# aff3ct/dvbs2

Measured on AMD Instinct MI355X. Metric: info_bits_per_s (N=64800 LDPC NMS 10-ite), higher is better.
Workload: dtype f32

## Files before the change

dvbs2_amd/csrc/dvbs2hip_api.hip:

```cpp
#include "dvbs2hip_handle.h"
#include "ldpc_dispatch.h"
#include "dvbs2_tables_gen.h"
#include <climits>
#include <new>

using namespace dvbs2;

namespace dvbs2 {
thread_local std::string g_create_error;

const char *modcod_name_by_pls(int b0_b6)
{
    for (int i = 0; i < DVBS2_N_MODCODS; i++) {
        int v = 0;
        for (int k = 0; k < 7; k++) v = v << 1 | (dvbs2_modcod_rows[i].pls[k] & 1);
        if (v == b0_b6) return dvbs2_modcod_rows[i].name;
    }
    return nullptr;
}

int pl_frame_by_pls(int b0_b6)
{
    for (int i = 0; i < DVBS2_N_MODCODS; i++) {
        const dvbs2_modcod_row &r = dvbs2_modcod_rows[i];
// ... 217 lines not shown
    const_cast<dvbs2hip_t *>(h)->ldpc_name = ldpc_choice_name(ldpc_choice(h, h->max_frames));
    return h->ldpc_name.c_str();
}

int dvbs2hip_reset(dvbs2hip_t *h)
{
    if (!h) return DVBS2HIP_EINVAL;
    int r = dvbs2hip_filter_reset(h);
    if (r) return r;
    if ((r = dvbs2hip_estimate_pilots_reset(h))) return r;
    if ((r = dvbs2hip_bbframe_reset(h))) return r;
    return dvbs2hip_monitor_reset(h);
}

int dvbs2hip_set_ldpc_params(dvbs2hip_t *h, int32_t n_ite, float alpha, int32_t early_stop)
{
    if (!h) return DVBS2HIP_EINVAL;
    if (n_ite < 1) return fail(h, DVBS2HIP_EINVAL, "'n_ite' has to be greater than 0");
    if (!(alpha > 0.f)) return fail(h, DVBS2HIP_EINVAL, "'alpha' has to be greater than 0");
    h->n_ite = n_ite; h->alpha = alpha; h->early_stop = early_stop ? 1 : 0;
    return 0;
}

void *dvbs2hip_get_stream(dvbs2hip_t *h) { return h ? (void *)h->stream : nullptr; }

int dvbs2hip_synchronize(dvbs2hip_t *h)
{
    int r0 = enter(h); if (r0) return r0;
    HIPCHK(h, hipStreamSynchronize(h->stream));
    return lr_check_all(h);
}

int dvbs2hip_graph_begin(dvbs2hip_t *h)
{
    int r0 = enter(h); if (r0) return r0;
    if (h->capturing) return fail(h, DVBS2HIP_EINVAL, "a capture is already open on this handle");
    if (h->timing) return fail(h, DVBS2HIP_EINVAL, "the per-kernel timers are on: their events cannot be recorded into a graph (dvbs2hip_timing_enable(h, 0) first)");
    HIPCHK(h, hipStreamBeginCapture(h->stream, hipStreamCaptureModeThreadLocal));
    h->capturing = true;
    return 0;
}

int dvbs2hip_graph_end(dvbs2hip_t *h, int32_t *graph)
{
    if (!h || !graph) return DVBS2HIP_EINVAL;
    if (!h->capturing) return fail(h, DVBS2HIP_EINVAL, "no capture is open on this handle");
// ... 25 lines not shown
    if (graph < 0 || (size_t)graph >= h->graphs.size() || !h->graphs[(size_t)graph]) return fail(h, DVBS2HIP_EINVAL, "unknown graph");
    (void)hipGraphExecDestroy(h->graphs[(size_t)graph]);
    h->graphs[(size_t)graph] = nullptr;
    return 0;
}

int dvbs2hip_get_sizes(const dvbs2hip_t *h, dvbs2hip_sizes *o)
{
    if (!h || !o) return DVBS2HIP_EINVAL;
    o->N_ldpc = h->N_ldpc; o->K_ldpc = h->K_ldpc; o->K_bch = h->K_bch; o->bps = h->bps;
    o->N_xfec_sym = h->n_sym; o->pl_frame_sym = h->pl_frame; o->ldpc_edges = h->ldpc.E; o->ldpc_q = h->ldpc.q;
    return 0;
}

static int ldpc_dev(dvbs2hip_t *h, const LdpcChoice &ch, const float *Y, int8_t *CWD, int32_t *V, uint32_t *packed, float *post, int32_t *ites, int F, int32_t *info_out = nullptr,
                    uint8_t *bch_flag = nullptr, int8_t *cwd_bch = nullptr)
{
    if (!ch.error.empty()) return fail(h, DVBS2HIP_EUNSUPPORTED, ch.error);
    LdpcKParams p;
    memset(&p, 0, sizeof p);
    p.llr = Y; p.bits = V; p.packed = packed; p.cwd = CWD; p.post = post; p.ites = ites; p.gwork = h->d_gwork;
    p.info_out = info_out; p.info_prbs = h->bch.d_prbs_rw; p.K_info = h->K_bch;
    if (info_out && bch_flag) { p.syn_tab = h->d_syn_pos; p.info_prbs_s = h->d_prbs_s; p.syn_words = h->syn_words; p.syn_rows = h->syn_rows; p.bch_flag = bch_flag; p.cwd_bch = cwd_bch; }
    p.n_frames = F; p.n_ite = h->n_ite; p.early_stop = h->early_stop; p.alpha = h->alpha;
    if (h->ldpc_sched == DVBS2HIP_SCHED_NATURAL) {
        LdpcPlan &pl = h->ldpc;
        if (!h->d_nat_work || !pl.d_nat_tab || !pl.d_nat_haz) {
            const size_t bytes = ((size_t)h->max_frames + 63) / 64 * ldpc_nat_group_words(pl) * sizeof(float);
            if (!h->d_nat_work && dev_alloc(h, &h->d_nat_work, bytes, "natural-order LDPC: workspace of " + std::to_string(bytes) + " bytes does not fit")) return DVBS2HIP_ENOMEM;
            if (!pl.d_nat_tab && upload(h, &pl.d_nat_tab, pl.nat_tab)) { (void)dev_free(h, &pl.d_nat_tab); return DVBS2HIP_EHIP; }
            if (!pl.d_nat_haz && upload(h, &pl.d_nat_haz, pl.nat_haz)) { (void)dev_free(h, &pl.d_nat_haz); return DVBS2HIP_EHIP; }
        }
    }
    Timer tm(h, DVBS2HIP_K_LDPC);
    if (ch.takes_order) {
        void *dord;
        int r = ensure(h, B_ORDER, (size_t)F * 8, &dord);
        if (r) return r;
        HIPCHK(h, frame_order_launch(Y, (float *)dord + F, (uint32_t *)dord, F, h->N_ldpc, h->stream));
        p.order = (const uint32_t *)dord;
    }
    HIPCHK(h, ldpc_launch(h->ldpc, ch, p, h->d_nat_work, h->stream));
    return 0;
}

int dvbs2hip_ldpc_decode_siho_dev(dvbs2hip_t *h, const float *Y_N, int8_t *CWD, int32_t *V_K, int32_t F)
{
// ... 356 lines not shown
```

dvbs2_amd/csrc/dvbs2hip_handle.h:

```cpp
#pragma once
#include "dvbs2hip_internal.h"
#include <cmath>
#include <cstdio>
#include <cstdlib>
#include <cstring>
#include <algorithm>
#include <map>
#include <utility>

namespace dvbs2 {

extern thread_local std::string g_create_error;

struct DevBuf {
    void *p = nullptr;
    size_t bytes = 0;
};

template <typename T>
struct PingPong {
    T *p[2] = {nullptr, nullptr};
    int cur = 0;
    T *in() const { return p[cur]; }
    T *out() const { return p[cur ^ 1]; }
    void flip() { cur ^= 1; }
};

}

struct dvbs2hip_handle {
    int N_ldpc = 0, K_ldpc = 0, K_bch = 0, bps = 0, itl_cols = 1, itl_order = 0;
    int n_sym = 0, pl_frame = 0, max_frames = 1, device = 0;
    int n_ite = 50, early_stop = 1, implem = 0;
    float alpha = 1.f, code_rate = 0.f;
    int fir_T = 0, fir_osf = 1;
    bool fir_sym = false;
    hipStream_t stream = nullptr;
    bool own_stream = false;
    bool capturing = false;
    bool lat_lds_ok = false;
    bool comm_dead = false;
    int red_timeout_ms = 0;
    std::vector<hipGraphExec_t> graphs;
    int n_cus = 256;
    dvbs2::LdpcPlan ldpc;
    dvbs2::BchPlan bch;
    float *d_cstl = nullptr;
    uint8_t *d_pl_seq = nullptr;
    float *d_taps_rev = nullptr;
    uint16_t *d_fir_afrag = nullptr, *d_upfir_afrag = nullptr;
    dvbs2::PingPong<float> d_hist;
    void *d_hist_all = nullptr;
    size_t hist_stride = 0;
    float *d_taps = nullptr;
    dvbs2::PingPong<float> d_uphist;
    unsigned long long *d_ctr = nullptr;
// ... 341 lines not shown
```

dvbs2_amd/csrc/dvbs2hip_internal.h:

```cpp
#pragma once
#include <hip/hip_runtime.h>
#include <stdint.h>
#include <string>
#include <vector>
#include "../../include/dvbs2hip.h"
#include "ldpc_layer_table.h"

namespace dvbs2 {

#if defined(__HIPCC__)
__device__ __forceinline__ float hw_exp(float x) { return __builtin_amdgcn_exp2f(x * 1.44269504088896341f); }
__device__ __forceinline__ float hw_log(float x) { return __builtin_amdgcn_logf(x) * 0.693147180559945309f; }
#endif

typedef uint32_t LdpcEntry;
enum { LE_T0_MASK = 0x1FF, LE_SLOT_SHIFT = 9, LE_SLOT_MASK = 0xFF, LE_LDS = 1u << 17, LE_MASK0 = 1u << 18,
       LE_LVL_SHIFT = 19, LE_LVL_MASK = 3, LE_NULL = 1u << 21 };

struct LdpcGroup {
    uint32_t base;
    uint32_t lds;
};

constexpr int LDPC_Z = 360;
// ... 8 lines not shown
    int8_t *cwd;
    float *post;
    int32_t *ites;
    int32_t *info_out;
    const uint32_t *info_prbs;
    int32_t K_info;
    const uint32_t *syn_tab;
    const uint32_t *info_prbs_s;
    int32_t syn_words;
    int32_t syn_rows;
    uint8_t *bch_flag;
    int8_t *cwd_bch;
    float *gwork;
    const LdpcEntry *entries;
    const int32_t *layer_deg;
    const int32_t *layer_lvl;
    const LdpcGroup *groups;
    int32_t N, K, M, q, n_info, n_groups;
    int32_t ent_stride;
    int32_t lds_post_words;
    int32_t glb_post_words;
    int32_t gwork_words;
    int32_t n_frames, n_ite, early_stop;
    float alpha;
    const uint32_t *order;
    float spa_cap;
    int32_t inf_row;
    uint32_t *cu_ctr;
    struct {
        const uint32_t *tab;
        const uint32_t *atab;
        const uint32_t *rows;
        uint32_t st_base;
        uint32_t lds_junk;
        int32_t lds_bytes, pad;
        int32_t nl_info, nl, ng_info, ng;
    } w8;
};

struct LdpcPlan {
    int N = 0, K = 0, M = 0, q = 0, n_info = 0, n_groups = 0, E = 0;
    int deg_max = 0, ent_stride = 0;
    int lds_groups = 0;
    bool c2v_lds = false, hybrid = false;
    int lds_post_words = 0, glb_post_words = 0, gwork_words = 0;
    size_t lds_bytes = 0;
// ... 10 lines not shown
    int spa_rule = 0;
    int fast_deg = 0;
    bool fast_pad = false;
    int fast_inf_row = -1;
    int fast_mode = 0;
    std::vector<uint32_t> nat_tab, nat_haz;
    uint32_t *d_nat_tab = nullptr, *d_nat_haz = nullptr;
    bool fast_cu1 = false;
    int cu1_pairs = 0;
    bool fast_wg8 = false;
    bool w8_dups_in_lds = false;
    std::vector<uint32_t> w8_tab, w8_rows;
    uint32_t *d_w8_tab = nullptr, *d_w8_rows = nullptr;
    std::vector<uint32_t> w8_atab;
    uint32_t *d_w8_atab = nullptr;
    uint32_t w8_st_base = 0, w8_lds_junk = 0;
    int w8_lds_bytes = 0, w8_gwork_words = 0, w8_nl_info = 0, w8_nl = 0, w8_ng_info = 0, w8_ng = 0;
    int w8_park_moves = 0;
    uint32_t *d_cu_ctr = nullptr;
};
constexpr int LDPC_PROF_WORDS = 1024 * 64;
constexpr int LDPC_CU_CTR_WORDS = 4096 + 64;
constexpr int LDPC_FRAME_CTR = 4096;
#ifndef LDPC_SPA_AT16_MAXDEG
#define LDPC_SPA_AT16_MAXDEG 13
#endif
constexpr int LDPC_AT_LANES = 384;
constexpr float LDPC_SPA_CAP = 16.6355324f;
constexpr int LDPC_FAST_MAXC = 16;
__host__ __device__ __forceinline__ constexpr int ldpc_park_nr(int mode) { return mode == 5 ? 39 : 32; }
__host__ __device__ __forceinline__ constexpr int ldpc_park_nl(int mode) { return mode == 5 ? 15 : 14; }
__host__ __device__ __forceinline__ constexpr int ldpc_w8_kd(int deg) { return deg == 27 ? 6 : deg == 11 ? 3 : deg == 13 ? 6 : deg; }
#ifndef LDPC_CU1_HA_V
#define LDPC_CU1_HA_V 14
#endif
constexpr int LDPC_CU1_HA = LDPC_CU1_HA_V;
constexpr int LDPC_CU1_XCHG_BYTES = 2 * LDPC_Z * 8;
__host__ __device__ __forceinline__ constexpr int ldpc_cu1_nrg() { return 36; }
#ifndef LDPC_CU1_DEFAULT
#define LDPC_CU1_DEFAULT 0
#endif
#ifndef LDPC_CU1_SPA_DEFAULT
#define LDPC_CU1_SPA_DEFAULT 1
#endif
constexpr int LDPC_W8_MISC_BYTES = 96;
constexpr int LDPC_SYN_RED = 640;
constexpr int LDPC_SPA_MAXC = 6;
constexpr int NAT_AHEAD = 24;
constexpr int NAT_HAZ_WINDOW = NAT_AHEAD + 1;
size_t ldpc_nat_group_words(const LdpcPlan &pl);
hipError_t ldpc_wg8_launch(const LdpcPlan &pl, LdpcKParams p, hipStream_t s);
int ldpc_wg8_blocks_per_cu(const LdpcPlan &pl);

std::string ldpc_build_plan(LdpcPlan &pl, int N, int K, int n_rows, const int32_t *row_ptr,
                            const int32_t *addr, int lds_groups_req, size_t lds_limit_bytes, int spa_rule = 0, bool small_batch = false);

struct BchPlan {
    int m = 0, n = 0, t = 0, N = 0, K = 0;
    std::vector<uint16_t> exp_, log_;
    uint16_t *d_exp = nullptr, *d_log = nullptr;
    uint32_t *d_prbs = nullptr;
    uint32_t *d_prbs_rw = nullptr;
    std::vector<uint16_t> syn_tab;
    uint16_t *d_syn_tab = nullptr;
};
struct BchKParams {
    const int32_t *in_bits;
    const uint32_t *in_packed;
// ... 156 lines not shown
```

dvbs2_amd/csrc/k_ldpc_wg8.hip:

```cpp
#include "dvbs2hip_internal.h"
#include "ldpc_layer_table.h"
#include "ldpc_device.h"
#include <cstdio>
#include <cstdlib>
#include <vector>
#include <algorithm>
#include <type_traits>

#include "ldpc_det.h"
namespace dvbs2 {

constexpr int W8_NL = 9;
constexpr int W8_IO = 16;
constexpr uint32_t W8_OOB = ATAB_DROPPED;
__host__ __device__ __forceinline__ constexpr bool w8_parked(int mode) { return mode == 4 || mode == 5; }
__host__ __device__ __forceinline__ constexpr bool w8_hybrid(int mode) { return mode == 3 || w8_parked(mode); }
__host__ __device__ __forceinline__ constexpr bool w8_slot_lds(int mode, int j) { return mode == 0 || (mode == 3 && j < W8_NL) || (w8_parked(mode) && j < ldpc_park_nl(mode)); }

constexpr int SPA_BS = 3;
#ifndef SPA_ABL
#define SPA_ABL 0
#endif
#ifndef W8_ABL
#define W8_ABL 0
// ... 3 lines not shown
#define PROF_MARK(i) do { if ((i) >= 6) LDPC_PROF_MARK(i); } while (0)
#define PROF_MARK_O(i) LDPC_PROF_MARK(i)
#else
#define PROF_MARK(i) LDPC_PROF_MARK(i)
#define PROF_MARK_O(i)
#endif
#else
#define PROF_MARK(i)
#define PROF_MARK_O(i)
#endif

__device__ __forceinline__ lds_float *w8_lds(uint32_t a) { return (lds_float *)(size_t)a; }

__device__ __forceinline__ int w8_lane_now()
{
    int l;
    asm volatile("v_mbcnt_lo_u32_b32 %0, -1, 0\n\tv_mbcnt_hi_u32_b32 %0, -1, %0" : "=v"(l));
    return l;
}

typedef float w8_f32x32 __attribute__((ext_vector_type(32)));

template <int DEG, int NR>
__device__ __forceinline__ void w8_park_server(const LdpcKParams &p, lds_int *const s_misc, const int wave, const int sidx)
{
    const int q = p.q;
    const const_u32 tab = (const_u32)p.w8.tab, srv = tab + q * LDPC_FAST_STRIDE;
    const const_u32 srow = (const_u32)p.w8.rows + p.w8.nl + p.w8.ng + q;
    const int lane = (int)threadIdx.x & 63, el = sidx * 64 + lane;
    const bool on = el < LDPC_Z / 3;
    const uint32_t a0 = (uint32_t)el * 4u;
    constexpr uint32_t A1 = LDPC_Z / 3 * 4u, A2 = 2u * A1;
    auto lst = [&](uint32_t a, float v) __attribute__((always_inline)) { *w8_lds(a) = v; };
    auto lxc = [&](uint32_t a, float v) __attribute__((always_inline)) -> float { return __hip_atomic_exchange(w8_lds(a), v, __ATOMIC_RELAXED, __HIP_MEMORY_SCOPE_WORKGROUP); };
    float R[NR][3];
    int nvote = 0;
    auto vote0 = [&]() __attribute__((always_inline)) -> bool {
        lds_int *const w = s_misc + 10;
        const int k = nvote % 3;
        nvote++;
        if (lane == 0 && wave == 0) w[(k + 1) % 3] = 0;
        __syncthreads();
        return w[k] != 0;
    };
    const const_u32 swm = srv + q * NR;
    auto moves = [&](int r) __attribute__((always_inline)) {
        const uint32_t mlo = swm[2 * r], mhi = swm[2 * r + 1];
// ... 24 lines not shown
        __syncthreads();
    };
    const bool es = p.early_stop != 0;
    for (int qp = blockIdx.x; qp < p.n_frames; ) {
        const int f = p.order ? (int)p.order[qp] : qp;
        const float *Y = p.llr + (size_t)f * p.N;
        const int eln = sidx * 64 + w8_lane_now();
        const int elc = eln < LDPC_Z / 3 ? eln : 0;
#pragma unroll
        for (int k = 0; k < NR; k++) {
            const uint32_t g = srow[k];
            const float *Yg = Y + (g == ROWS_NONE ? 0u : g) * (uint32_t)LDPC_Z;
            R[k][0] = __builtin_nontemporal_load(&Yg[elc]); R[k][1] = __builtin_nontemporal_load(&Yg[elc + LDPC_Z / 3]); R[k][2] = __builtin_nontemporal_load(&Yg[elc + 2 * (LDPC_Z / 3)]);
        }
        __syncthreads();
        int ph = 0, r = 0, it = 0;
        bool ok = false, fin = false;
        while (!fin) {
            bool mv = true;
            if (ph == 1 && es && r == 0 && vote0()) { ok = false; mv = false; ph = 3; }
            if (mv) moves(r);
            if (ph == 0) {
                layer_barriers(r);
                if (++r == q) { r = 0; it++; if (es || it == p.n_ite) { ph = 1; ok = true; } }
            } else if (ph == 1) {
                bool bad = false;
                if (es) { if (r == 0) __syncthreads(); else bad = vote0(); }
                else { if (r == q - 1) { if (vote0()) ok = false; } else __syncthreads(); }
                if (bad) { ok = false; ph = 2; }
                if (++r == q) { if (ph == 2) __syncthreads(); ph = 3; }
            } else if (ph == 2) {
                if (++r == q) { __syncthreads(); ph = 3; }
            }
            if (ph == 3) { if (ok || it >= p.n_ite) fin = true; else { ph = 0; r = 0; } }
        }
        __syncthreads();
#pragma unroll
        for (int k = 0; k < NR; k++) if (on) { const uint32_t b = (uint32_t)k * (uint32_t)LDPC_ROW; lst(b + a0, R[k][0]); lst(b + a0 + A1, R[k][1]); lst(b + a0 + A2, R[k][2]); }
        __syncthreads();
        __syncthreads();
        qp = s_misc[9];
    }
}

template <int DEG, int MODE, int SPA = 0>
__global__ void __launch_bounds__(512) __attribute__((amdgpu_waves_per_eu((SPA == 2 && DEG > 13) ? 2 : 4, 4)))
ldpc_wg8_kernel(const LdpcKParams p)
// ... 16 lines not shown
    __syncthreads();
    int role;
    {
        int k = 0, c0 = 0, c1 = 0, c2 = 0, c3 = 0;
        for (int w = 0; w < 8; w++) {
            const int s = s_misc[w];
            c0 += s == 0; c1 += s == 1; c2 += s == 2; c3 += s == 3;
            if (w < wave && s == simd) k++;
        }
        const bool balanced = c0 == 2 && c1 == 2 && c2 == 2 && c3 == 2;
        if (!balanced) role = wave < 6 ? wave : -1;
        else if (k == 0) role = simd;
        else role = ((simd >> 1) == s_misc[8]) ? 4 + (simd & 1) : -1;
        role = __builtin_amdgcn_readfirstlane(role);
        if (w8_parked(MODE) && role < 0) {
            int sidx = 0;
            for (int w = 0; w < wave; w++) {
                const int s = s_misc[w];
                int kw = 0;
                for (int w2 = 0; w2 < w; w2++) kw += s_misc[w2] == s;
                const int rw = !balanced ? (w < 6 ? w : -1) : kw == 0 ? s : ((s >> 1) == s_misc[8] ? 4 + (s & 1) : -1);
                sidx += rw < 0;
            }
            w8_park_server<DEG, ldpc_park_nr(MODE)>(p, s_misc, wave, __builtin_amdgcn_readfirstlane(sidx));
#ifdef LDPC_PHASE_PROF
            if (lane0 == 0 && p.cu_ctr) for (int i = 0; i < 12; i++) p.cu_ctr[LDPC_CU_CTR_WORDS + ((int)blockIdx.x * 8 + wave) * 12 + i] = 0u;
#endif
            return;
        }
    }
    const int lane = w8_lane_now() & 63;
    const int t = role * 64 + lane;
    const bool act = role >= 0 && t < LDPC_Z;
    const uint32_t t4 = (uint32_t)t * 4u;
    const int q = p.q, M = p.M;
    float *gwork = p.gwork + (size_t)blockIdx.x * p.gwork_words;
    const __amdgpu_buffer_rsrc_t rs = __builtin_amdgcn_make_buffer_rsrc(gwork, 0, p.gwork_words * 4, 0x00020000);
    const const_u32 tab = (const_u32)p.w8.tab;
    const const_u32 rows = (const_u32)p.w8.rows;
    const uint32_t st_base = p.w8.st_base;
    const uint32_t ljunk = p.w8.lds_junk;
    uint32_t SB = 0x80000000u;
    asm volatile("" : "+s"(SB));
    auto wide_off = [&](uint32_t voff, uint32_t soff) __attribute__((always_inline)) -> uint32_t { uint32_t o = voff + soff; asm volatile("" : "+v"(o)); return o; };
    auto gld = [&](uint32_t voff, uint32_t soff) __attribute__((always_inline)) { return __builtin_bit_cast(float, __builtin_amdgcn_raw_buffer_load_b32(rs, voff, soff, 0)); };
    auto gst = [&](uint32_t voff, uint32_t soff, float v) __attribute__((always_inline)) { __builtin_amdgcn_raw_buffer_store_b32(__builtin_bit_cast(uint32_t, v), rs, voff, soff, 0); };
    auto gld1 = [&](uint32_t voff, uint32_t soff) __attribute__((always_inline)) { if (W8_ABL & 2) { float r; asm volatile("v_mov_b32 %0, %1" : "=v"(r) : "v"(voff | 0x3F000000u)); return r; } return gld(voff, soff); };
// ... 13 lines not shown
            dst[4 * g] = __uint_as_float(v.x); dst[4 * g + 1] = __uint_as_float(v.y); dst[4 * g + 2] = __uint_as_float(v.z); dst[4 * g + 3] = __uint_as_float(v.w);
        }
        const uint32_t tbase = lbase + (uint32_t)MG4 * (LDPC_ROW * 4u);
        if (MR == 3) { m_u32x3 v = {0u, 0u, 0u}; if (!(SPA_ABL & 2)) v = __builtin_amdgcn_raw_buffer_load_b96(rs, tb * 3u, tbase, 0);
                       dst[4 * MG4] = __uint_as_float(v.x); dst[4 * MG4 + 1] = __uint_as_float(v.y); dst[4 * MG4 + 2] = __uint_as_float(v.z); }
        if (MR == 2) { m_u32x2 v = {0u, 0u}; if (!(SPA_ABL & 2)) v = __builtin_amdgcn_raw_buffer_load_b64(rs, tb * 2u, tbase, 0);
                       dst[4 * MG4] = __uint_as_float(v.x); dst[4 * MG4 + 1] = __uint_as_float(v.y); }
        if (MR == 1) dst[4 * MG4] = mld(tb, tbase);
    };
    auto mone_ld = [&](uint32_t slot, uint32_t tb, uint32_t lbase) __attribute__((always_inline)) -> float {
        const uint32_t g = slot >> 2, k = slot & 3u;
        return g < (uint32_t)MG4 ? mld(tb * 4u, lbase + g * (LDPC_ROW * 4u) + k * 4u) : mld(tb * (uint32_t)(MR ? MR : 1), lbase + (uint32_t)MG4 * (LDPC_ROW * 4u) + k * 4u);
    };
    auto lld = [&](uint32_t a) __attribute__((always_inline)) -> float { return *w8_lds(a); };
    auto lst = [&](uint32_t a, float v) __attribute__((always_inline)) { *w8_lds(a) = v; };
    const int nl_info = p.w8.nl_info, nl = p.w8.nl, ng_info = p.w8.ng_info, ng = p.w8.ng;
    const uint32_t grow0 = 2u * LDPC_ROW;
    constexpr bool ATAB = !SPA && MODE == 0;
    constexpr bool AT16 = SPA && MODE == 0 && DEG <= LDPC_SPA_AT16_MAXDEG;
    constexpr int ND16 = (DEG + 1) / 2, NP16 = (ND16 + 3) / 4;
    const __amdgpu_buffer_rsrc_t rs_at = __builtin_amdgcn_make_buffer_rsrc((void *)((ATAB || AT16) ? p.w8.atab : (const uint32_t *)p.w8.tab), 0, ATAB ? p.q * ((DEG + 3) / 4) * (LDPC_AT_LANES * 16) : AT16 ? p.q * NP16 * (LDPC_AT_LANES * 16) : 0, 0x00020000);
    const uint32_t at_vo = (uint32_t)(role >= 0 ? t : 0) * 16u;
    constexpr bool FWD = w8_hybrid(MODE);
#ifdef LDPC_PHASE_PROF
    uint32_t prof[12];
    for (int i = 0; i < 12; i++) prof[i] = 0u;
    const unsigned long long prof_t0 = __builtin_amdgcn_s_memtime();
    unsigned long long pt_ = prof_t0;
#endif

    for (int qp = blockIdx.x; qp < p.n_frames; ) {
        const int f = p.order ? (int)__builtin_amdgcn_readfirstlane((int)p.order[qp]) : qp;
        const float *Y = p.llr + (size_t)f * p.N;
        constexpr bool INF = MODE == 0;
        const int lio = (SPA || INF) ? w8_lane_now() : lane, tio = (SPA || INF) ? role * 64 + lio : t;
        const uint32_t tio4 = (SPA || INF) ? (uint32_t)tio * 4u : t4;
        __builtin_amdgcn_s_setprio(3);
        if (INF && act) {
            const int fin = __builtin_amdgcn_readfirstlane(f);
            const __amdgpu_buffer_rsrc_t rs_llr = __builtin_amdgcn_make_buffer_rsrc((void *)(p.llr + (size_t)fin * p.N), 0, p.N * 4, 0x00020000);
            auto in_body = [&](int rb, int l0, bool lds, auto b_c) __attribute__((always_inline)) {
                constexpr int B = decltype(b_c)::value;
                float v[B];
#pragma unroll
                for (int k = 0; k < B; k++) v[k] = __builtin_bit_cast(float, __builtin_amdgcn_raw_buffer_load_b32(rs_llr, tio4, rows[rb + l0 + k] * (uint32_t)LDPC_ROW, 2));
#pragma unroll
// ... 33 lines not shown
            const int dq = 64 / q, dr = 64 - dq * q;
            int tl = lio / q, r = lio - tl * q;
            constexpr int PIO = 8;
            for (int i0 = 0; i0 < q; i0 += PIO) {
                float v[PIO];
#pragma unroll
                for (int k = 0; k < PIO; k++) { const int e = (i0 + k) * 64 + lio; v[k] = e < cnt ? Yp[e] : 0.f; }
#pragma unroll
                for (int k = 0; k < PIO; k++) {
                    if ((i0 + k) * 64 + lio < cnt) {
                        const uint32_t loc = prow[r], off = (loc & ~ROWS_GLOBAL) + (uint32_t)(tl0 + tl) * 4u;
                        if (loc >> ROWS_GLOBAL_BIT) gst(off, 0u, v[k]); else lst(off, v[k]);
                    }
                    tl += dq; r += dr;
                    if (r >= q) { r -= q; tl++; }
                }
            }
        }
        if (act) {
            if (p.w8.pad) { if (MODE == 0) lst(ljunk + LDPC_ROW + t4, INFINITY); else gst(t4, LDPC_ROW, INFINITY); }
            if (AT16 && t == 0) lst(ljunk + 4u, INFINITY);
        }
        if (p.packed && (SPA ? wave == 0 && lio == 0 : threadIdx.x == 0) && (p.K & 31)) p.packed[(size_t)f * ((p.K + 31) / 32) + p.K / 32] = 0u;
        __builtin_amdgcn_s_setprio(0);
        __syncthreads();
        PROF_MARK(8);

        int it = 0;
        bool ok = false;
        float nx1 = 0.f, nx2 = 0.f, nxk = 0.f;
        float pfw = 0.f;
        float onx[SPA ? DEG : 1];
#pragma unroll
        for (int j = 0; j < (SPA ? DEG : 1); j++) onx[j] = 0.f;
        uint32_t TE[32];
#pragma unroll
        for (int j = 0; j < 32; j++) TE[j] = tab[j];
        constexpr int NW4 = (DEG + 3) / 4;
        uint32_t w[4 * NW4];
        auto at_request = [&](int rl) __attribute__((always_inline)) {
            typedef uint32_t at_u32x4 __attribute__((ext_vector_type(4)));
#pragma unroll
            for (int g4 = 0; g4 < NW4; g4++) {
                const uint32_t so = (uint32_t)((rl * NW4 + g4) * (LDPC_AT_LANES * 16));
                const at_u32x4 q4 = __builtin_amdgcn_raw_buffer_load_b128(rs_at, at_vo, so, 0); w[4 * g4] = q4.x; w[4 * g4 + 1] = q4.y; w[4 * g4 + 2] = q4.z; w[4 * g4 + 3] = q4.w;
            }
// ... 238 lines not shown
                    }
                    {
                        const const_u32 Tn = tab + (r + 1 < q ? r + 1 : 0) * LDPC_FAST_STRIDE;
#pragma unroll
                        for (int j = 0; j < 32; j++) TE[j] = Tn[j];
                    }
                    __syncthreads();
                    continue;
                }
                float v[DEG];
                constexpr bool EARLY_B1 = MODE == 0;
                static_assert(LDPC_Z > 64 * 5 && LDPC_Z <= 64 * 6, "six working waves, the last one with active lanes (EARLY_B1's barrier sits inside `if (act)`)");
                constexpr bool ABSF = MODE == 0, SGNA = MODE == 0;
                constexpr int KD = MODE == 0 ? ldpc_w8_kd(DEG) : DEG;
                constexpr bool DREG = MODE == 0;
                constexpr int KDD = ldpc_w8_kd(DEG);
                float dold[KDD];
#pragma unroll
                for (int j = 0; j < KDD; j++) dold[j] = 0.f;
                const float c1o = nx1, c2o = nx2;
                const uint32_t pko = __float_as_uint(nxk);
                float mn1 = INFINITY, mn2 = INFINITY, cst1 = 0.f, cst2 = 0.f;
                uint32_t sacc = 0u, tot = 0u, pkn = 0u;
                if (EARLY_B1 && ncf > 0 && role < 0) asm volatile("s_barrier" ::: "memory");
                if (act) {
                    __builtin_amdgcn_s_setprio(3);
#pragma unroll
                    for (int j = 0; j < DEG; j++) {
                        const uint32_t base = (E[j] >> LT_BASE_SHIFT) & LT_BASE_MASK;
                        if (ATAB) {
                            v[j] = lld(w[j]);
                            continue;
                        }
                        const uint32_t d = t4 - (E[j] & LT_SHIFT_MASK);
                        w[j] = min(d, d + (uint32_t)LDPC_ROW);
                        if (FWD && j == DEG - 1) { if (r > 0) v[j] = pfw; else v[j] = gld1(w[j], base); }
                        else if (w8_slot_lds(MODE, j)) {
                            const uint32_t a = w[j] + base;
                            v[j] = lld(a);
                            if (j >= KD) w[j] = a;
                        } else v[j] = gld1(w[j], base);
                    }
                    const int rn = r + 1 < q ? r + 1 : 0;
                    if (it == 0 && r + 1 < q) { nx1 = 0.f; nx2 = 0.f; nxk = 0.f; }
                    else {
                        typedef uint32_t u32x3 __attribute__((ext_vector_type(3)));
// ... 16 lines not shown
                            sacc = __builtin_amdgcn_alignbit(sacc, __float_as_uint(x), 31);
                        }
                    } else {
                    uint32_t psh = pko << (32u - DEG);
#pragma unroll
                    for (int j = 0; j < DEG; j++) {
                        const float mag = (idxo == (uint32_t)j) ? c1o : c2o;
                        const float old = and_or(SGNA ? psh : pko << ((32u - DEG) + j), SB, mag);
                        if (SGNA && j + 1 < DEG) asm("v_add_u32_e32 %0, %0, %0" : "+v"(psh));
                        if (DREG && j < KDD) dold[j] = old;
                        float x = v[j] - old;
                        if (j == DEG - 1 && mask0) x = INFINITY;
                        v[j] = x;
                        const float a = fabsf(x);
                        if (W8_ABL & 4) { if (j == 0) { mn1 = a; mn2 = a + 1.f; sacc = __float_as_uint(x); } continue; }
                        mn2 = __builtin_amdgcn_fmed3f(mn1, mn2, a);
                        if (ABSF) asm("v_min_f32_e64 %0, %0, |%1|" : "+v"(mn1) : "v"(x)); else mn1 = fminf(mn1, a);
                        sacc = __builtin_amdgcn_alignbit(sacc, __float_as_uint(x), 31);
                    }
                    }
                    cst1 = mn2 * p.alpha; cst2 = mn1 * p.alpha;
                    tot = (uint32_t)(__popc(sacc) & 1);
                    pkn = sacc ^ (tot ? ((1u << DEG) - 1u) : 0u);
                }
                PROF_MARK(1);
                if (!EARLY_B1 && ncf > 0) __syncthreads();
                PROF_MARK(2);
                if (act) {
                    __builtin_amdgcn_s_setprio(MODE == 0 ? 3 : 2);
                    uint32_t idxn = 0u;
                    float m1s = __uint_as_float(__float_as_uint(cst1) | (tot << 31));
                    float m2s = __uint_as_float(__float_as_uint(cst2) | (tot << 31));
                    asm volatile("" : "+v"(m1s), "+v"(m2s));
                    constexpr int P2_ROT = w8_hybrid(MODE) ? (MODE == 3 ? W8_NL : ldpc_park_nl(MODE)) : 0;
#pragma unroll
                    for (int jj = 0; jj < DEG; jj++) {
                        const int j = jj + P2_ROT < DEG ? jj + P2_ROT : jj + P2_ROT - DEG;
                        const float x = v[j];
                        const bool ismin = (W8_ABL & 8) ? j == 3 : fabsf(x) == mn1;
                        const float mag = ismin ? m1s : m2s;
                        const float nw = __uint_as_float(__float_as_uint(mag) ^ (__float_as_uint(x) & SB));
                        idxn = ismin ? (uint32_t)j : idxn;
                        asm("" : "+v"(idxn));
                        if (DREG && j < KDD) dold[j] = nw - dold[j];
                        const bool pr = ((prim >> j) & 1u) != 0u;
                        const uint32_t base = (E[j] >> LT_BASE_SHIFT) & LT_BASE_MASK;
// ... 24 lines not shown
                if (ATAB && role >= 0) {
                    __builtin_amdgcn_sched_barrier(0);
                    at_request(r + 1 < q ? r + 1 : 0);
                    __builtin_amdgcn_sched_barrier(0);
                }
                PROF_MARK(3);
                if (ncf > 0) {
                    auto addr_of = [&](uint32_t e) __attribute__((always_inline)) { const uint32_t d = t4 - (e & LT_SHIFT_MASK); return min(d, d + (uint32_t)LDPC_ROW); };
                    auto delta_of = [&](uint32_t j) __attribute__((always_inline)) { return ldpc_unpack<DEG>(cst1, cst2, pkn, j, SB) - ldpc_unpack<DEG>(c1o, c2o, pko, j, SB); };
                    const uint32_t j0 = (cinfo >> LT_CINFO_SLOT0_SHIFT) & LT_SLOT_MASK, j1 = (cinfo >> LT_CINFO_SLOT1_SHIFT) & LT_SLOT_MASK, lvl1 = (cinfo >> LT_CINFO_LVL1_SHIFT) & LT_LVL_MASK;
                    const bool two = ncf > 1 && lvl1 == 1u;
                    uint32_t o0 = 0, b0 = 0, o1 = 0, b1 = 0;
                    float d0 = 0.f, d1 = 0.f;
                    if (DREG) { o0 = addr_of(ce0); b0 = (ce0 >> LT_BASE_SHIFT) & LT_BASE_MASK; o1 = addr_of(ce1); b1 = (ce1 >> LT_BASE_SHIFT) & LT_BASE_MASK; d0 = dold[0]; d1 = dold[KDD > 1 ? 1 : 0]; }
                    __syncthreads();
                    if (act) {
                        if (!DREG) { o0 = addr_of(ce0); b0 = (ce0 >> LT_BASE_SHIFT) & LT_BASE_MASK; o1 = addr_of(ce1); b1 = (ce1 >> LT_BASE_SHIFT) & LT_BASE_MASK; d0 = delta_of(j0); d1 = delta_of(j1); }
                        float L0, L1 = 0.f;
                        if (MODE != 1) { L0 = lld(o0 + b0); if (two) L1 = lld(o1 + b1); }
                        else { L0 = gld(o0, b0); if (two) L1 = gld(o1, b1); }
                        const float n0 = L0 + d0, n1 = L1 + d1;
                        if (MODE != 1) { lst(o0 + b0, n0); if (two) lst(o1 + b1, n1); }
                        else { gst(o0, b0, n0); if (two) gst(o1, b1, n1); }
                    }
                    uint32_t prev_lvl = 1u;
                    if (DREG) {
#pragma unroll
                        for (int i = 1; i < KDD; i++) {
                            if (i < (two ? 2 : 1) || i >= ncf) continue;
                            const uint32_t e = T[LT_CONF + i], lvl = T[LT_CONF_META + i] >> LT_META_LVL_SHIFT;
                            const uint32_t off = addr_of(e), base = (e >> LT_BASE_SHIFT) & LT_BASE_MASK;
                            if (lvl != prev_lvl) { __syncthreads(); prev_lvl = lvl; }
                            if (act) { const float Lv = lld(off + base); lst(off + base, Lv + dold[i]); }
                        }
                    } else
                    for (int i = two ? 2 : 1; i < ncf; i++) {
                        const uint32_t e = T[LT_CONF + i], meta = T[LT_CONF_META + i];
                        const uint32_t j = meta & LT_SLOT_MASK, lvl = meta >> LT_META_LVL_SHIFT;
                        if (lvl != prev_lvl) { __syncthreads(); prev_lvl = lvl; }
                        if (act) {
                            const uint32_t off = addr_of(e), base = (e >> LT_BASE_SHIFT) & LT_BASE_MASK;
                            if (MODE != 1) { const float Lv = lld(off + base); lst(off + base, Lv + delta_of(j)); }
                            else { const float Lv = gld(off, base); gst(off, base, Lv + delta_of(j)); }
                        }
                    }
                }
                PROF_MARK(4);
                {
                    const const_u32 Tn = tab + (r + 1 < q ? r + 1 : 0) * LDPC_FAST_STRIDE;
#pragma unroll
                    for (int j = 0; j < 32; j++) TE[j] = Tn[j];
                }
                __syncthreads();
                PROF_MARK(5);
            }
            it++;
            if (p.early_stop || it == p.n_ite) {
                ok = true;
                int bad = 0;
                auto vote = [&](int b) __attribute__((always_inline)) -> bool {
                    const bool any = __ballot(b != 0) != 0ull;
                    lds_int *const w = s_misc + 10;
                    const int k = nvote % 3;
                    nvote++;
                    if (w8_lane_now() == 0) { if (any) w[k] = 1; if (wave == 0) w[(k + 1) % 3] = 0; }
                    __syncthreads();
                    return w[k] != 0;
                };
                for (int r = 0; r < q; r++) {
                    if (act) {
                        const const_u32 T = tab + r * LDPC_FAST_STRIDE;
                        float Lv[DEG];
#pragma unroll
                        for (int j = 0; j < DEG; j++) {
                            const uint32_t e = T[j];
                            const uint32_t d = t4 - (e & LT_SHIFT_MASK);
                            const uint32_t wo = min(d, d + (uint32_t)LDPC_ROW), base = (e >> LT_BASE_SHIFT) & LT_BASE_MASK;
                            Lv[j] = w8_slot_lds(MODE, j) ? lld(wo + base) : gld(wo, base);
                        }
                        if (r == 0 && t == 0) Lv[DEG - 1] = 0.f;
                        uint32_t x = 0u;
#pragma unroll
                        for (int j = 0; j < DEG; j++) x ^= __float_as_uint(Lv[j]);
                        bad |= (int)(x >> 31);
                    }
                    if (w8_parked(MODE)) {
                        if (p.early_stop) {
                            if (vote(bad)) { ok = false; if (r > 0) __syncthreads(); break; }
                            if (r == 0) __syncthreads();
                        } else if (r == q - 1) { if (vote(bad)) ok = false; }
                        else __syncthreads();
                        continue;
// ... 348 lines not shown
```

dvbs2_amd/lib_binding.py:

```python
from __future__ import annotations

import ctypes as C
import os

from . import build as _build

_lib = None


class Dvbs2HipError(RuntimeError):
    def __init__(self, code, msg):
        super().__init__("dvbs2hip error %d: %s" % (code, msg))
        self.code = code


class Cfg(C.Structure):
    _fields_ = [
        ("N_ldpc", C.c_int32), ("K_ldpc", C.c_int32), ("K_bch", C.c_int32),
        ("ldpc_n_rows", C.c_int32), ("ldpc_row_ptr", C.c_void_p), ("ldpc_addr", C.c_void_p),
        ("ldpc_n_ite", C.c_int32), ("ldpc_implem", C.c_int32), ("ldpc_alpha", C.c_float),
        ("ldpc_early_stop", C.c_int32),
        ("bch_m", C.c_int32), ("bch_t", C.c_int32), ("bch_prim", C.c_void_p),
        ("bps", C.c_int32), ("cstl", C.c_void_p),
        ("itl_cols", C.c_int32), ("itl_order", C.c_int32),
# ... 49 lines not shown
    "dvbs2hip_pls_scan_dev": (C.c_int, [_vp, _vp, _i, _vp, _vp, _vp]),
    "dvbs2hip_pls_search": (C.c_int, [_vp, _vp, _i, _vp, _vp, _vp]),
    "dvbs2hip_pls_search_dev": (C.c_int, [_vp, _vp, _i, _vp, _vp, _vp]),
    "dvbs2hip_pls_frame_symbols": (C.c_int, [_i]),
    "dvbs2hip_pls_walk": (C.c_int, [_vp, _vp, _i, _i, _vp, _f, _i, _vp, _vp, _vp, _vp, _vp, _vp]),
    "dvbs2hip_pls_walk_dev": (C.c_int, [_vp, _vp, _i, _i, _vp, _f, _i, _vp, _vp, _vp, _vp, _vp, _vp, _vp]),
    "dvbs2hip_estimate_pilots": (C.c_int, [_vp, _vp, _i, _vp, _vp, _vp, _i]),
    "dvbs2hip_estimate_pilots_dev": (C.c_int, [_vp, _vp, _i, _vp, _vp, _vp, _i]),
    "dvbs2hip_estimate_pilots_located_dev": (C.c_int, [_vp, _vp, _i, _vp, _vp, _vp, _i]),
    "dvbs2hip_estimate_pilots_set_alpha": (C.c_int, [_vp, _f]),
    "dvbs2hip_estimate_pilots_reset": (C.c_int, [_vp]),
    "dvbs2hip_bbframe_set_params": (C.c_int, [_vp, _i, _i, _i, _i, _i]),
    "dvbs2hip_bbframe_reset": (C.c_int, [_vp]),
    "dvbs2hip_bbframe_get_stats": (C.c_int, [_vp, _vp]),
    "dvbs2hip_bbframe_max_packets": (C.c_int, [_vp, _i, C.POINTER(C.c_int32)]),
    "dvbs2hip_bbframe_build": (C.c_int, [_vp, _vp, C.c_int64, _vp, _i]),
    "dvbs2hip_bbframe_build_dev": (C.c_int, [_vp, _vp, C.c_int64, _vp, _i]),
    "dvbs2hip_bbframe_parse": (C.c_int, [_vp, _vp, _vp, _vp, _vp, _vp, _vp, _i]),
    "dvbs2hip_bbframe_parse_dev": (C.c_int, [_vp, _vp, _vp, _vp, _vp, _vp, _vp, _i]),
    "dvbs2hip_rx_bb_up": (C.c_int, [_vp, _vp, _vp, _vp, _vp, _vp, _vp, _vp, _vp, _i]),
    "dvbs2hip_rx_bb_up_dev": (C.c_int, [_vp, _vp, _vp, _vp, _vp, _vp, _vp, _vp, _vp, _i]),
    "dvbs2hip_sync_frame_get_metric": (C.c_int, [_vp, C.POINTER(C.c_float), C.POINTER(C.c_int32)]),
    "dvbs2hip_set_ldpc_params": (C.c_int, [_vp, _i, _f, _i]),
    "dvbs2hip_get_stream": (_vp, [_vp]),
    "dvbs2hip_synchronize": (C.c_int, [_vp]),
    "dvbs2hip_graph_begin": (C.c_int, [_vp]),
    "dvbs2hip_graph_end": (C.c_int, [_vp, C.POINTER(C.c_int32)]),
    "dvbs2hip_graph_launch": (C.c_int, [_vp, _i]),
    "dvbs2hip_graph_destroy": (C.c_int, [_vp, _i]),
    "dvbs2hip_get_sizes": (C.c_int, [_vp, C.POINTER(Sizes)]),
    "dvbs2hip_ldpc_decode_siho": (C.c_int, [_vp, _vp, _vp, _vp, _i]),
    "dvbs2hip_ldpc_decode_siho_dev": (C.c_int, [_vp, _vp, _vp, _vp, _i]),
    "dvbs2hip_ldpc_decode_siho_post": (C.c_int, [_vp, _vp, _vp, _vp, _vp, _vp, _i]),
    "dvbs2hip_bch_decode_hiho": (C.c_int, [_vp, _vp, _vp, _vp, _i]),
    "dvbs2hip_bch_decode_hiho_dev": (C.c_int, [_vp, _vp, _vp, _vp, _i]),
    "dvbs2hip_demodulate": (C.c_int, [_vp, _vp, _vp, _vp, _i]),
    "dvbs2hip_demodulate_dev": (C.c_int, [_vp, _vp, _vp, _vp, _i]),
    "dvbs2hip_deinterleave": (C.c_int, [_vp, _vp, _vp, _i]),
    "dvbs2hip_deinterleave_dev": (C.c_int, [_vp, _vp, _vp, _i]),
    "dvbs2hip_demodulate_deinterleave": (C.c_int, [_vp, _vp, _vp, _vp, _i]),
    "dvbs2hip_demodulate_deinterleave_dev": (C.c_int, [_vp, _vp, _vp, _vp, _i]),
    "dvbs2hip_filter": (C.c_int, [_vp, _vp, _vp, _i, _i]),
    "dvbs2hip_filter_dev": (C.c_int, [_vp, _vp, _vp, _i, _i]),
    "dvbs2hip_filter_reset": (C.c_int, [_vp]),
    "dvbs2hip_filter_split": (C.c_int, [_vp, _i]),
    "dvbs2hip_filter1": (C.c_int, [_vp, _vp, _vp, _i, _i]),
# ... 114 lines not shown
```

dvbs2_amd/receiver.py:

```python
from __future__ import annotations

import ctypes as C

import numpy as np

from . import lib_binding as B
from . import params as P


def _ptr(a):
    if a is None:
        return None
    if isinstance(a, int):
        return C.c_void_p(a)
    return a.ctypes.data_as(C.c_void_p)


class Dvbs2Hip:
    def __init__(self, modcod: str = "QPSK-S_8/9", max_frames: int = 1, n_ite: int = 50, alpha: float = 1.0,
                 early_stop: bool = True, device: int = 0, stream: int | None = None, fir_taps=None,
                 fir_osf: int = 2, lds_groups: int = -1, implem: str = "NMS"):
        self.L = B.load()
        self.h = None
        self.mc = P.get_modcod(modcod)
# ... 42 lines not shown
            self.close()
        except Exception:
            pass

    def _frames(self, a, per_frame, dtype):
        a = np.ascontiguousarray(a, dtype=dtype)
        if a.size % per_frame:
            raise ValueError("socket size %d is not a multiple of the frame size %d" % (a.size, per_frame))
        return a.reshape(-1, per_frame), a.size // per_frame

    @property
    def stream(self) -> int:
        return int(self.L.dvbs2hip_get_stream(self.h) or 0)

    def synchronize(self):
        self._chk(self.L.dvbs2hip_synchronize(self.h))

    def reset(self):
        self._chk(self.L.dvbs2hip_reset(self.h))

    def set_ldpc_params(self, n_ite, alpha=1.0, early_stop=True):
        self._chk(self.L.dvbs2hip_set_ldpc_params(self.h, int(n_ite), float(alpha), 1 if early_stop else 0))

    def host_register(self, arr):
        self._chk(self.L.dvbs2hip_host_register(self.h, _ptr(arr), arr.nbytes))

    def host_unregister(self, arr):
        self._chk(self.L.dvbs2hip_host_unregister(self.h, _ptr(arr)))

    def decode_siho(self, Y_N, with_post=False, out=None):
        Y, F = self._frames(Y_N, self.N_ldpc, np.float32)
        if out is not None:
            V, CWD = out
            assert V.dtype == np.int32 and V.size == F * self.K_ldpc and CWD.dtype == np.int8 and CWD.size == F and V.flags.c_contiguous
        else:
            V = np.empty((F, self.K_ldpc), dtype=np.int32)
            CWD = np.zeros(F, dtype=np.int8)
        if not with_post:
            self._chk(self.L.dvbs2hip_ldpc_decode_siho(self.h, _ptr(Y), _ptr(CWD), _ptr(V), F))
            return V, CWD
        post = np.empty((F, self.N_ldpc), dtype=np.float32)
        ites = np.zeros(F, dtype=np.int32)
        self._chk(self.L.dvbs2hip_ldpc_decode_siho_post(self.h, _ptr(Y), _ptr(CWD), _ptr(V), _ptr(post), _ptr(ites), F))
        return V, CWD, post, ites

    def decode_siho_dev(self, Y_N, CWD, V_K, n_frames):
# ... 610 lines not shown
```

include/dvbs2hip.h:

```cpp
#ifndef DVBS2HIP_H
#define DVBS2HIP_H

#include <stddef.h>
#include <stdint.h>

#ifdef __cplusplus
extern "C" {
#endif

#define DVBS2HIP_VERSION 101

typedef enum {
    DVBS2HIP_OK           = 0,
    DVBS2HIP_EINVAL       = -1,
    DVBS2HIP_ENOMEM       = -2,
    DVBS2HIP_EHIP         = -3,
    DVBS2HIP_EUNSUPPORTED = -4,
    DVBS2HIP_ENODEVICE    = -5,
    DVBS2HIP_ETIMEOUT     = -6
} dvbs2hip_status;

typedef struct dvbs2hip_handle dvbs2hip_t;

enum { DVBS2HIP_IMPLEM_NMS = 0, DVBS2HIP_IMPLEM_MS = 1,
// ... 23 lines not shown
    int32_t itl_cols;
    int32_t itl_order;
    int32_t      fir_n_taps;
    const float *fir_taps;
    int32_t      fir_osf;
    int32_t max_frames;
    int32_t device;
    void   *stream;
    int32_t ldpc_lds_groups;
    int32_t pls[7];
} dvbs2hip_cfg;

int dvbs2hip_cfg_from_modcod(const char *modcod, dvbs2hip_cfg *cfg);
int dvbs2hip_create(const dvbs2hip_cfg *cfg, dvbs2hip_t **out);
int dvbs2hip_device_count(int32_t *count);
void dvbs2hip_destroy(dvbs2hip_t *h);
const char *dvbs2hip_last_error(const dvbs2hip_t *h);
int dvbs2hip_set_ldpc_schedule(dvbs2hip_t *h, int32_t schedule);
const char *dvbs2hip_ldpc_kernel_name(const dvbs2hip_t *h);
int dvbs2hip_host_register(dvbs2hip_t *h, void *ptr, size_t bytes);
int dvbs2hip_host_unregister(dvbs2hip_t *h, void *ptr);
int dvbs2hip_reset(dvbs2hip_t *h);
int dvbs2hip_set_ldpc_params(dvbs2hip_t *h, int32_t n_ite, float alpha, int32_t early_stop);
void *dvbs2hip_get_stream(dvbs2hip_t *h);
int dvbs2hip_synchronize(dvbs2hip_t *h);
int dvbs2hip_graph_begin(dvbs2hip_t *h);
int dvbs2hip_graph_end(dvbs2hip_t *h, int32_t *graph);
int dvbs2hip_graph_launch(dvbs2hip_t *h, int32_t graph);
int dvbs2hip_graph_destroy(dvbs2hip_t *h, int32_t graph);
typedef struct dvbs2hip_sizes {
    int32_t N_ldpc, K_ldpc, K_bch, bps, N_xfec_sym, pl_frame_sym, ldpc_edges, ldpc_q;
} dvbs2hip_sizes;
int dvbs2hip_get_sizes(const dvbs2hip_t *h, dvbs2hip_sizes *out);

int dvbs2hip_ldpc_decode_siho(dvbs2hip_t *h, const float *Y_N, int8_t *CWD, int32_t *V_K, int32_t n_frames);
int dvbs2hip_ldpc_decode_siho_dev(dvbs2hip_t *h, const float *Y_N, int8_t *CWD, int32_t *V_K, int32_t n_frames);
int dvbs2hip_ldpc_decode_siho_post(dvbs2hip_t *h, const float *Y_N, int8_t *CWD, int32_t *V_K,
                                   float *post_N, int32_t *n_ite_done, int32_t n_frames);

int dvbs2hip_bch_decode_hiho(dvbs2hip_t *h, const int32_t *Y_N, int8_t *CWD, int32_t *V_K, int32_t n_frames);
int dvbs2hip_bch_decode_hiho_dev(dvbs2hip_t *h, const int32_t *Y_N, int8_t *CWD, int32_t *V_K, int32_t n_frames);

int dvbs2hip_demodulate(dvbs2hip_t *h, const float *CP, const float *Y_N1, float *Y_N2, int32_t n_frames);
int dvbs2hip_demodulate_dev(dvbs2hip_t *h, const float *CP, const float *Y_N1, float *Y_N2, int32_t n_frames);

int dvbs2hip_deinterleave(dvbs2hip_t *h, const float *itl, float *nat, int32_t n_frames);
// ... 185 lines not shown
```

Before: 40.86 billion.

## Skip final syndrome sweep when last iteration proves codeword stable

During the last decoding iteration with early stop off, the min-sum layered kernel sets a shared-memory flag whenever a check node is unsatisfied or any posterior LLR changes sign. If no flag is raised, all checks held at the start of their layer and no hard decision moved afterwards, so the codeword is certified valid. In that case the final q-layer syndrome verification sweep is skipped, and a device counter records how often that happens. The cost is extra compare-and-store work in the hot last-iteration update loops, plus a new default-on option and API.

```diff
diff --git a/dvbs2_amd/csrc/dvbs2hip_api.hip b/dvbs2_amd/csrc/dvbs2hip_api.hip
--- a/dvbs2_amd/csrc/dvbs2hip_api.hip
+++ b/dvbs2_amd/csrc/dvbs2hip_api.hip
@@ -263,6 +263,24 @@
     return 0;
 }
 
+int dvbs2hip_set_ldpc_cert(dvbs2hip_t *h, int32_t on)
+{
+    if (!h) return DVBS2HIP_EINVAL;
+    h->ldpc_cert = on ? 1 : 0;
+    return 0;
+}
+
+int dvbs2hip_ldpc_cert_skipped(dvbs2hip_t *h, uint32_t *skipped)
+{
+    int r0 = enter(h); if (r0) return r0;
+    if (!skipped) return fail(h, DVBS2HIP_EINVAL, "null pointer");
+    *skipped = 0u;
+    if (!h->ldpc.d_cu_ctr) return 0;
+    HIPCHK(h, hipStreamSynchronize(h->stream));
+    HIPCHK(h, hipMemcpy(skipped, h->ldpc.d_cu_ctr + LDPC_CERT_CTR, sizeof(uint32_t), hipMemcpyDeviceToHost));
+    return 0;
+}
+
 void *dvbs2hip_get_stream(dvbs2hip_t *h) { return h ? (void *)h->stream : nullptr; }
 
 int dvbs2hip_synchronize(dvbs2hip_t *h)
@@ -334,7 +352,7 @@
     p.llr = Y; p.bits = V; p.packed = packed; p.cwd = CWD; p.post = post; p.ites = ites; p.gwork = h->d_gwork;
     p.info_out = info_out; p.info_prbs = h->bch.d_prbs_rw; p.K_info = h->K_bch;
     if (info_out && bch_flag) { p.syn_tab = h->d_syn_pos; p.info_prbs_s = h->d_prbs_s; p.syn_words = h->syn_words; p.syn_rows = h->syn_rows; p.bch_flag = bch_flag; p.cwd_bch = cwd_bch; }
-    p.n_frames = F; p.n_ite = h->n_ite; p.early_stop = h->early_stop; p.alpha = h->alpha;
+    p.n_frames = F; p.n_ite = h->n_ite; p.early_stop = h->early_stop; p.alpha = h->alpha; p.cert = h->ldpc_cert;
     if (h->ldpc_sched == DVBS2HIP_SCHED_NATURAL) {
         LdpcPlan &pl = h->ldpc;
         if (!h->d_nat_work || !pl.d_nat_tab || !pl.d_nat_haz) {
diff --git a/dvbs2_amd/csrc/dvbs2hip_handle.h b/dvbs2_amd/csrc/dvbs2hip_handle.h
--- a/dvbs2_amd/csrc/dvbs2hip_handle.h
+++ b/dvbs2_amd/csrc/dvbs2hip_handle.h
@@ -32,6 +32,7 @@
     int N_ldpc = 0, K_ldpc = 0, K_bch = 0, bps = 0, itl_cols = 1, itl_order = 0;
     int n_sym = 0, pl_frame = 0, max_frames = 1, device = 0;
     int n_ite = 50, early_stop = 1, implem = 0;
+    int ldpc_cert = 1;
     float alpha = 1.f, code_rate = 0.f;
     int fir_T = 0, fir_osf = 1;
     bool fir_sym = false;
diff --git a/dvbs2_amd/csrc/dvbs2hip_internal.h b/dvbs2_amd/csrc/dvbs2hip_internal.h
--- a/dvbs2_amd/csrc/dvbs2hip_internal.h
+++ b/dvbs2_amd/csrc/dvbs2hip_internal.h
@@ -54,6 +54,7 @@
     int32_t glb_post_words;
     int32_t gwork_words;
     int32_t n_frames, n_ite, early_stop;
+    int32_t cert;
     float alpha;
     const uint32_t *order;
     float spa_cap;
@@ -110,6 +111,7 @@
 constexpr int LDPC_PROF_WORDS = 1024 * 64;
 constexpr int LDPC_CU_CTR_WORDS = 4096 + 64;
 constexpr int LDPC_FRAME_CTR = 4096;
+constexpr int LDPC_CERT_CTR = 4097;
 #ifndef LDPC_SPA_AT16_MAXDEG
 #define LDPC_SPA_AT16_MAXDEG 13
 #endif
@@ -132,6 +134,7 @@
 #define LDPC_CU1_SPA_DEFAULT 1
 #endif
 constexpr int LDPC_W8_MISC_BYTES = 96;
+constexpr int LDPC_W8_CERT = 13;
 constexpr int LDPC_SYN_RED = 640;
 constexpr int LDPC_SPA_MAXC = 6;
 constexpr int NAT_AHEAD = 24;
diff --git a/dvbs2_amd/csrc/k_ldpc_wg8.hip b/dvbs2_amd/csrc/k_ldpc_wg8.hip
--- a/dvbs2_amd/csrc/k_ldpc_wg8.hip
+++ b/dvbs2_amd/csrc/k_ldpc_wg8.hip
@@ -49,7 +49,7 @@
 typedef float w8_f32x32 __attribute__((ext_vector_type(32)));
 
 template <int DEG, int NR>
-__device__ __forceinline__ void w8_park_server(const LdpcKParams &p, lds_int *const s_misc, const int wave, const int sidx)
+__device__ __forceinline__ void w8_park_server(const LdpcKParams &p, lds_int *const s_misc, const int wave, const int sidx, const bool cert)
 {
     const int q = p.q;
     const const_u32 tab = (const_u32)p.w8.tab, srv = tab + q * LDPC_FAST_STRIDE;
@@ -120,7 +120,13 @@
             if (mv) moves(r);
             if (ph == 0) {
                 layer_barriers(r);
-                if (++r == q) { r = 0; it++; if (es || it == p.n_ite) { ph = 1; ok = true; } }
+                if (++r == q) {
+                    r = 0; it++;
+                    if (es || it == p.n_ite) {
+                        ph = 1; ok = true;
+                        if (cert && __builtin_amdgcn_readfirstlane(s_misc[LDPC_W8_CERT]) == 0) ph = 3;
+                    }
+                }
             } else if (ph == 1) {
                 bool bad = false;
                 if (es) { if (r == 0) __syncthreads(); else bad = vote0(); }
@@ -183,7 +189,7 @@
                 const int rw = !balanced ? (w < 6 ? w : -1) : kw == 0 ? s : ((s >> 1) == s_misc[8] ? 4 + (s & 1) : -1);
                 sidx += rw < 0;
             }
-            w8_park_server<DEG, ldpc_park_nr(MODE)>(p, s_misc, wave, __builtin_amdgcn_readfirstlane(sidx));
+            w8_park_server<DEG, ldpc_park_nr(MODE)>(p, s_misc, wave, __builtin_amdgcn_readfirstlane(sidx), !SPA && p.cert != 0 && p.early_stop == 0);
 #ifdef LDPC_PHASE_PROF
             if (lane0 == 0 && p.cu_ctr) for (int i = 0; i < 12; i++) p.cu_ctr[LDPC_CU_CTR_WORDS + ((int)blockIdx.x * 8 + wave) * 12 + i] = 0u;
 #endif
@@ -243,6 +249,7 @@
     const __amdgpu_buffer_rsrc_t rs_at = __builtin_amdgcn_make_buffer_rsrc((void *)((ATAB || AT16) ? p.w8.atab : (const uint32_t *)p.w8.tab), 0, ATAB ? p.q * ((DEG + 3) / 4) * (LDPC_AT_LANES * 16) : AT16 ? p.q * NP16 * (LDPC_AT_LANES * 16) : 0, 0x00020000);
     const uint32_t at_vo = (uint32_t)(role >= 0 ? t : 0) * 16u;
     constexpr bool FWD = w8_hybrid(MODE);
+    const bool cert = !SPA && p.cert != 0 && p.early_stop == 0;
 #ifdef LDPC_PHASE_PROF
     uint32_t prof[12];
     for (int i = 0; i < 12; i++) prof[i] = 0u;
@@ -322,6 +329,7 @@
             if (AT16 && t == 0) lst(ljunk + 4u, INFINITY);
         }
         if (p.packed && (SPA ? wave == 0 && lio == 0 : threadIdx.x == 0) && (p.K & 31)) p.packed[(size_t)f * ((p.K + 31) / 32) + p.K / 32] = 0u;
+        if (!SPA && threadIdx.x == 0) s_misc[LDPC_W8_CERT] = 0;
         __builtin_amdgcn_s_setprio(0);
         __syncthreads();
         PROF_MARK(8);
@@ -606,6 +614,7 @@
                 const uint32_t pko = __float_as_uint(nxk);
                 float mn1 = INFINITY, mn2 = INFINITY, cst1 = 0.f, cst2 = 0.f;
                 uint32_t sacc = 0u, tot = 0u, pkn = 0u;
+                const bool cert_last = cert && it + 1 == p.n_ite;
                 if (EARLY_B1 && ncf > 0 && role < 0) asm volatile("s_barrier" ::: "memory");
                 if (act) {
                     __builtin_amdgcn_s_setprio(3);
@@ -668,6 +677,7 @@
                     cst1 = mn2 * p.alpha; cst2 = mn1 * p.alpha;
                     tot = (uint32_t)(__popc(sacc) & 1);
                     pkn = sacc ^ (tot ? ((1u << DEG) - 1u) : 0u);
+                    if (cert_last && (tot | ((pko ^ sacc) & ((1u << DEG) - 1u))) != 0u) s_misc[LDPC_W8_CERT] = 1;
                 }
                 PROF_MARK(1);
                 if (!EARLY_B1 && ncf > 0) __syncthreads();
@@ -738,6 +748,7 @@
                         const float n0 = L0 + d0, n1 = L1 + d1;
                         if (MODE != 1) { lst(o0 + b0, n0); if (two) lst(o1 + b1, n1); }
                         else { gst(o0, b0, n0); if (two) gst(o1, b1, n1); }
+                        if (cert_last && (((__float_as_uint(n0) ^ __float_as_uint(L0)) | (two ? __float_as_uint(n1) ^ __float_as_uint(L1) : 0u)) >> 31) != 0u) s_misc[LDPC_W8_CERT] = 1;
                     }
                     uint32_t prev_lvl = 1u;
                     if (DREG) {
@@ -747,7 +758,11 @@
                             const uint32_t e = T[LT_CONF + i], lvl = T[LT_CONF_META + i] >> LT_META_LVL_SHIFT;
                             const uint32_t off = addr_of(e), base = (e >> LT_BASE_SHIFT) & LT_BASE_MASK;
                             if (lvl != prev_lvl) { __syncthreads(); prev_lvl = lvl; }
-                            if (act) { const float Lv = lld(off + base); lst(off + base, Lv + dold[i]); }
+                            if (act) {
+                                const float Lv = lld(off + base), nv = Lv + dold[i];
+                                lst(off + base, nv);
+                                if (cert_last && ((__float_as_uint(nv) ^ __float_as_uint(Lv)) >> 31) != 0u) s_misc[LDPC_W8_CERT] = 1;
+                            }
                         }
                     } else
                     for (int i = two ? 2 : 1; i < ncf; i++) {
@@ -756,8 +771,9 @@
                         if (lvl != prev_lvl) { __syncthreads(); prev_lvl = lvl; }
                         if (act) {
                             const uint32_t off = addr_of(e), base = (e >> LT_BASE_SHIFT) & LT_BASE_MASK;
-                            if (MODE != 1) { const float Lv = lld(off + base); lst(off + base, Lv + delta_of(j)); }
-                            else { const float Lv = gld(off, base); gst(off, base, Lv + delta_of(j)); }
+                            const float Lv = MODE != 1 ? lld(off + base) : gld(off, base), nv = Lv + delta_of(j);
+                            if (MODE != 1) lst(off + base, nv); else gst(off, base, nv);
+                            if (cert_last && ((__float_as_uint(nv) ^ __float_as_uint(Lv)) >> 31) != 0u) s_misc[LDPC_W8_CERT] = 1;
                         }
                     }
                 }
@@ -774,6 +790,9 @@
             if (p.early_stop || it == p.n_ite) {
                 ok = true;
                 int bad = 0;
+                const bool skip = cert && __builtin_amdgcn_readfirstlane(s_misc[LDPC_W8_CERT]) == 0;
+                if (skip && wave == 0 && w8_lane_now() == 0 && p.cu_ctr) atomicAdd(&p.cu_ctr[LDPC_CERT_CTR], 1u);
+                const int q_sweep = skip ? 0 : q;
                 auto vote = [&](int b) __attribute__((always_inline)) -> bool {
                     const bool any = __ballot(b != 0) != 0ull;
                     lds_int *const w = s_misc + 10;
@@ -783,7 +802,7 @@
                     __syncthreads();
                     return w[k] != 0;
                 };
-                for (int r = 0; r < q; r++) {
+                for (int r = 0; r < q_sweep; r++) {
                     if (act) {
                         const const_u32 T = tab + r * LDPC_FAST_STRIDE;
                         float Lv[DEG];
diff --git a/dvbs2_amd/lib_binding.py b/dvbs2_amd/lib_binding.py
--- a/dvbs2_amd/lib_binding.py
+++ b/dvbs2_amd/lib_binding.py
@@ -95,6 +95,8 @@
     "dvbs2hip_rx_bb_up_dev": (C.c_int, [_vp, _vp, _vp, _vp, _vp, _vp, _vp, _vp, _vp, _i]),
     "dvbs2hip_sync_frame_get_metric": (C.c_int, [_vp, C.POINTER(C.c_float), C.POINTER(C.c_int32)]),
     "dvbs2hip_set_ldpc_params": (C.c_int, [_vp, _i, _f, _i]),
+    "dvbs2hip_set_ldpc_cert": (C.c_int, [_vp, _i]),
+    "dvbs2hip_ldpc_cert_skipped": (C.c_int, [_vp, C.POINTER(C.c_uint32)]),
     "dvbs2hip_get_stream": (_vp, [_vp]),
     "dvbs2hip_synchronize": (C.c_int, [_vp]),
     "dvbs2hip_graph_begin": (C.c_int, [_vp]),
diff --git a/dvbs2_amd/receiver.py b/dvbs2_amd/receiver.py
--- a/dvbs2_amd/receiver.py
+++ b/dvbs2_amd/receiver.py
@@ -88,6 +88,14 @@
     def set_ldpc_params(self, n_ite, alpha=1.0, early_stop=True):
         self._chk(self.L.dvbs2hip_set_ldpc_params(self.h, int(n_ite), float(alpha), 1 if early_stop else 0))
 
+    def set_ldpc_cert(self, on=True):
+        self._chk(self.L.dvbs2hip_set_ldpc_cert(self.h, 1 if on else 0))
+
+    def ldpc_cert_skipped(self) -> int:
+        n = C.c_uint32(0)
+        self._chk(self.L.dvbs2hip_ldpc_cert_skipped(self.h, C.byref(n)))
+        return int(n.value)
+
     def host_register(self, arr):
         self._chk(self.L.dvbs2hip_host_register(self.h, _ptr(arr), arr.nbytes))
 
diff --git a/include/dvbs2hip.h b/include/dvbs2hip.h
--- a/include/dvbs2hip.h
+++ b/include/dvbs2hip.h
@@ -69,6 +69,8 @@
 int dvbs2hip_host_unregister(dvbs2hip_t *h, void *ptr);
 int dvbs2hip_reset(dvbs2hip_t *h);
 int dvbs2hip_set_ldpc_params(dvbs2hip_t *h, int32_t n_ite, float alpha, int32_t early_stop);
+int dvbs2hip_set_ldpc_cert(dvbs2hip_t *h, int32_t on);
+int dvbs2hip_ldpc_cert_skipped(dvbs2hip_t *h, uint32_t *skipped);
 void *dvbs2hip_get_stream(dvbs2hip_t *h);
 int dvbs2hip_synchronize(dvbs2hip_t *h);
 int dvbs2hip_graph_begin(dvbs2hip_t *h);
```

Result: no change. 41.26 billion, median of 6 (+1.0%).
